# Bebra777228/PolGen-RVC

Hardware: AMD Instinct MI355X
Metric: real-time-factor (audio-sec/wall-sec) per GPU, 30s@16kHz RMVPE->48kHz (higher is better)
Workload: dtype f32 (conv products as 3 fp16 MFMAs of a hi/lo split, fp32 accumulate; fp32 elsewhere)

## Files before the change

polgen-rvc_amd/csrc/api_ops.hip:

```cpp
#include "api_internal.h"
#include "h3_device.h"

using namespace rvcx;
using namespace rvcx::api;

static void to_host(Ctx& c, float* h, const float* d, size_t n) {
  RVCX_HIP(hipMemcpyAsync(h, d, n * sizeof(float), hipMemcpyDeviceToHost, c.stream));
  RVCX_HIP(hipStreamSynchronize(c.stream));
}
#define TEMP_REGION(C) WeightRegion tmp_region_; RegionScope tmp_scope_(*(C), tmp_region_)

extern "C" {

int rvcx_op_conv1d(rvcx_ctx* ctx, const float* x, const float* w, const float* bias, const float* res,
                   float* y, int B, int Cin, int Tin, int Cout, int K, int stride, int dil,
                   int pad_left, int Tout, int groups, int pre_lrelu, float pre_slope, int act,
                   float act_slope, const int32_t* lens_in, const int32_t* lens_out) {
  API_BEGIN(ctx)
  TEMP_REGION(C);
  size_t nx = (size_t)B * Cin * Tin, ny = (size_t)B * Cout * Tout;
  C->arena.reserve((nx + 2 * ny) * 4 + (64 << 20));
  C->arena.reset();
  ConvW L = make_conv(*C, w, bias, Cout, Cin / groups, K, groups, true);
  float* dx = to_dev(*C, x, nx);
// ... 409 lines not shown
  for (size_t r = 0; r < (size_t)B * Cout * 2 * H; ++r)
    if (yp[r * Wpo] != 0.f || yp[r * Wpo + Wpo - 1] != 0.f) fail("convT2d: pad column not zero");
  unpad_rows(yp, y, (size_t)B * Cout, 2 * H, 2 * W);
  C->arena.reset();
  API_END
}

int rvcx_op_attention(rvcx_ctx* ctx, const float* q, const float* k, const float* v, float* out, int B, int H,
                      int D, int T, float scale, const float* emb_rel_k, const float* emb_rel_v, int window,
                      const int32_t* lens) {
  API_BEGIN(ctx)
  const size_t n = (size_t)B * H * D * T;
  C->arena.reserve(n * 16 + (attention_scratch_floats(B, H, T, window) + attention_split_floats(B, H, T)) * 4 + (64 << 20));
  C->arena.reset();
  float *dq = to_dev(*C, q, n), *dk = to_dev(*C, k, n), *dv = to_dev(*C, v, n);
  float* dout = C->arena.alloc<float>(n);
  float *ek = nullptr, *ev = nullptr, *scratch = nullptr;
  if (emb_rel_k) {
    ek = to_dev(*C, emb_rel_k, (size_t)(2 * window + 1) * D);
    ev = to_dev(*C, emb_rel_v, (size_t)(2 * window + 1) * D);
    scratch = C->arena.alloc<float>(attention_scratch_floats(B, H, T, window));
  }
  launch_attention(dq, dk, dv, dout, B, H, D, T, T, (long)H * D * T, (long)H * D * T, scale, ek, ev, window,
                   (lens ? to_dev(*C, lens, B) : nullptr), scratch, C->arena.alloc<float>(attention_split_floats(B, H, T)), C->stream);
  to_host(*C, out, dout, n);
  C->arena.reset();
  API_END
}

static void decode_xs(const std::vector<uint16_t>& raw, long rows, int Cc, float* out) {
  for (long r = 0; r < rows; ++r)
    for (int c = 0; c < Cc; ++c) {
      const size_t e = ((size_t)r * Cc * 2) + (size_t)(c >> 4) * 32 + ((c >> 3) & 1) * 8 + (c & 7);
      out[(size_t)r * Cc + c] = half_to_float(raw[e]) + half_to_float(raw[e + 16]) / 256.f;
    }
}

static void decode_split_cf(const std::vector<uint16_t>& raw, int B, int Cc, int T, float* out) {
  for (int b = 0; b < B; ++b)
    for (int c = 0; c < Cc; ++c)
      for (int t = 0; t < T; ++t) {
        const size_t item = (size_t)b * Cc * T * 2;
        const size_t hi = item + ((size_t)(((c >> 4) * 2 + 0) * 2 + ((c >> 3) & 1)) * T + t) * 8 + (c & 7);
        const size_t lo = item + ((size_t)(((c >> 4) * 2 + 1) * 2 + ((c >> 3) & 1)) * T + t) * 8 + (c & 7);
        out[((size_t)b * Cc + c) * T + t] = half_to_float(raw[hi]) + half_to_float(raw[lo]) / kH3Scale;
      }
}
// ... 445 lines not shown
```

polgen-rvc_amd/csrc/attention.hip:

```cpp
#include <cstdlib>

#include "conv.h"
#include "conv_device.h"
#include "ops.h"

namespace rvcx {

constexpr int KT = 32;
constexpr int VROW = 33;

template <int DT>
__global__ __launch_bounds__(256) void attn_kernel(const float* __restrict__ q, const float* __restrict__ k,
                                                   const float* __restrict__ v, float* __restrict__ out,
                                                   float* __restrict__ m_out, float* __restrict__ l_out,
                                                   const float* __restrict__ relq, int H, int D, int T,
                                                   int ld, long in_bs, long out_bs, float scale, int window,
                                                   const int* lens, int nsplit, float* opart) {
  __shared__ float Ks[32 * DT * KT];
  __shared__ float Vs[32 * DT * VROW];
  const int tid = threadIdx.x, lane = tid & 63, wave = tid >> 6;
  const int i = lane & 31, h = lane >> 5;
  const int b = blockIdx.z, hd = blockIdx.y;
  const int qblk = blockIdx.x / nsplit, split = blockIdx.x - qblk * nsplit;
  const int q0 = qblk * 128 + wave * 32;
  const int len = lens ? lens[b] : T;
  const long base = (long)b * in_bs + (long)hd * D * ld;
  const long obase = (long)b * out_bs + (long)hd * D * ld;
  const float* qb = q + base;
  const float* kb = k + base;
  const float* vb = v + base;
  const int nsteps = D / 2;

  float qreg[16 * DT];
  const int qi = q0 + i;
#pragma unroll
  for (int s = 0; s < 16 * DT; ++s) {
    float val = 0.f;
    if (s < nsteps && qi < T) val = qb[(long)(2 * s + h) * ld + qi] * scale;
    qreg[s] = val;
  }

  f32x16 acc_o[DT];
#pragma unroll
  for (int dt = 0; dt < DT; ++dt)
#pragma unroll
    for (int r = 0; r < 16; ++r) acc_o[dt][r] = 0.f;
  float m_run = -INFINITY, l_run = 0.f;
  const int nrel = 2 * window + 1;
  const float* relrow = relq ? relq + (((long)b * H + hd) * T + min(qi, T - 1)) * nrel : nullptr;

  const int tiles = (len + KT - 1) / KT;
  const int klo = (int)((long)tiles * split / nsplit) * KT;
  const int khi = min(len, (int)((long)tiles * (split + 1) / nsplit) * KT);
  for (int k0 = klo; k0 < khi; k0 += KT) {
    __syncthreads();
    for (int idx = tid; idx < 32 * DT * KT; idx += 256) {
      const int d = idx / KT, kk = idx % KT;
      const int key = k0 + kk;
      float kv = 0.f, vv = 0.f;
      if (d < D && key < len) {
        kv = kb[(long)d * ld + key];
        vv = vb[(long)d * ld + key];
      }
      Ks[d * KT + kk] = kv;
      Vs[d * VROW + kk] = vv;
    }
    __syncthreads();
    f32x16 sacc;
#pragma unroll
    for (int r = 0; r < 16; ++r) sacc[r] = 0.f;
#pragma unroll
    for (int s = 0; s < 16 * DT; ++s) {
      if (s < nsteps) {
        const float a = Ks[(2 * s + h) * KT + i];
        sacc = __builtin_amdgcn_mfma_f32_32x32x2f32(a, qreg[s], sacc, 0, 0, 0);
      }
    }
    const bool band = relq && (k0 <= q0 + 31 + window) && (k0 + KT - 1 >= q0 - window);
    float mloc = -INFINITY;
#pragma unroll
    for (int r = 0; r < 16; ++r) {
      const int key = k0 + (r & 3) + 8 * (r >> 2) + 4 * h;
      float sv = sacc[r];
      if (band) {
        const int rel = key - qi + window;
        if (rel >= 0 && rel < nrel && qi < T) sv += relrow[rel];
      }
      if (key >= len) sv = -INFINITY;
      sacc[r] = sv;
      mloc = fmaxf(mloc, sv);
    }
    const float mtile = fmaxf(mloc, __shfl_xor(mloc, 32));
    const float m_new = fmaxf(m_run, mtile);
    const float alpha = (m_run == -INFINITY) ? 0.f : expf(m_run - m_new);
    float lloc = 0.f;
#pragma unroll
    for (int r = 0; r < 16; ++r) {
      const float p = (sacc[r] == -INFINITY) ? 0.f : expf(sacc[r] - m_new);
      sacc[r] = p;
      lloc += p;
    }
    l_run = l_run * alpha + lloc + __shfl_xor(lloc, 32);
    m_run = m_new;
#pragma unroll
    for (int dt = 0; dt < DT; ++dt)
#pragma unroll
      for (int r = 0; r < 16; ++r) acc_o[dt][r] *= alpha;
#pragma unroll
    for (int s = 0; s < 16; ++s) {
      const int kidx = (s & 3) + 8 * (s >> 2) + 4 * h;
#pragma unroll
      for (int dt = 0; dt < DT; ++dt) {
        const float a = Vs[(dt * 32 + i) * VROW + kidx];
        acc_o[dt] = __builtin_amdgcn_mfma_f32_32x32x2f32(a, sacc[s], acc_o[dt], 0, 0, 0);
      }
    }
  }
  if (nsplit > 1) {
    if (qi < T) {
      const int DP = 32 * DT;
      float* pb = opart + (((long)b * H + hd) * nsplit + split) * (DP + 2) * T;
#pragma unroll
      for (int dt = 0; dt < DT; ++dt)
#pragma unroll
        for (int r = 0; r < 16; ++r) {
          const int d = dt * 32 + (r & 3) + 8 * (r >> 2) + 4 * h;
          pb[(long)d * T + qi] = acc_o[dt][r];
        }
      if (h == 0) {
        pb[(long)DP * T + qi] = m_run;
        pb[(long)(DP + 1) * T + qi] = l_run;
      }
    }
    return;
  }
  if (qi < T) {
    const float inv = 1.f / l_run;
    float* ob = out + obase;
#pragma unroll
    for (int dt = 0; dt < DT; ++dt)
#pragma unroll
      for (int r = 0; r < 16; ++r) {
        const int d = dt * 32 + (r & 3) + 8 * (r >> 2) + 4 * h;
        if (d < D) ob[(long)d * ld + qi] = (qi < len) ? acc_o[dt][r] * inv : 0.f;
      }
    if (m_out && h == 0) {
      m_out[((long)b * H + hd) * T + qi] = m_run;
      l_out[((long)b * H + hd) * T + qi] = l_run;
    }
  }
}

typedef _Float16 ahalf8 __attribute__((ext_vector_type(8)));
constexpr float kAttS = 256.f;
#ifndef RVCX_ATT_ABL
#define RVCX_ATT_ABL 0
#endif
constexpr int kAttAbl = RVCX_ATT_ABL;
__device__ __forceinline__ f32x16 att_mfma(ahalf8 a, ahalf8 b, f32x16 c) {
#if defined(__HIP_DEVICE_COMPILE__)
  return __builtin_amdgcn_mfma_f32_32x32x16_f16(a, b, c, 0, 0, 0);
#else
  return c;
#endif
}

struct AttRsrc {
#if defined(__HIP_DEVICE_COMPILE__)
  __amdgpu_buffer_rsrc_t r;
#endif
};
__device__ __forceinline__ AttRsrc att_rsrc(const float* base, int bytes) {
  AttRsrc b;
#if defined(__HIP_DEVICE_COMPILE__)
  b.r = __builtin_amdgcn_make_buffer_rsrc(const_cast<float*>(base), 0, bytes, 0x00020000);
#endif
  return b;
}
__device__ __forceinline__ float att_load(const AttRsrc& b, int off) {
#if defined(__HIP_DEVICE_COMPILE__)
  return __builtin_bit_cast(float, __builtin_amdgcn_raw_buffer_load_b32(b.r, off, 0, 0));
// ... 35 lines not shown
    ko[((s * 2 + 1) * 2 + hh) * 32 + key] = __builtin_bit_cast(uint4, a2);
  }
  for (int e0 = tid; e0 < V_ELEMS; e0 += 256) {
    const int dd = e0 & 31, hh = (e0 >> 5) & 1, s2 = (e0 >> 6) & 1, dt = e0 >> 7;
    const int d = dt * 32 + dd;
    ahalf8 a0, a2;
#pragma unroll
    for (int e = 0; e < 8; ++e) {
      const int r = 8 * s2 + e;
      const int key = k0 + (r & 3) + 8 * (r >> 2) + 4 * hh;
      const float val = (d < D && key < len) ? vb[(long)d * ld + key] : 0.f;
      ovf |= !(fabsf(val) < kH3ActLimit / kAttS);
      const _Float16 vh = (_Float16)val;
      a0[e] = (_Float16)((float)vh * kAttS);
      a2[e] = (_Float16)((val - (float)vh) * kAttS);
    }
    vo[(((dt * 2 + s2) * 2 + 0) * 2 + hh) * 32 + dd] = __builtin_bit_cast(uint4, a0);
    vo[(((dt * 2 + s2) * 2 + 1) * 2 + hh) * 32 + dd] = __builtin_bit_cast(uint4, a2);
  }
  if (ovf) report_h3_overflow(ovf_word, ovf_layer, seq);
}

typedef unsigned att_u32x4 __attribute__((ext_vector_type(4)));
template <int NKE, int NVE>
__device__ __forceinline__ void att_fetch(att_u32x4 (&rk)[NKE], att_u32x4 (&rv)[NVE], const uint4* __restrict__ kp,
                                          const uint4* __restrict__ vp, int tid) {
#pragma unroll
  for (int j = 0; j < NKE; ++j) rk[j] = *reinterpret_cast<const att_u32x4*>(kp + tid + 256 * j);
#pragma unroll
  for (int j = 0; j < NVE; ++j) rv[j] = *reinterpret_cast<const att_u32x4*>(vp + tid + 256 * j);
}
template <int NKE, int NVE>
__device__ __forceinline__ void att_commit(const att_u32x4 (&rk)[NKE], const att_u32x4 (&rv)[NVE], uint4* Ks, uint4* Vs,
                                           int tid) {
#pragma unroll
  for (int j = 0; j < NKE; ++j) *reinterpret_cast<att_u32x4*>(Ks + tid + 256 * j) = rk[j];
#pragma unroll
  for (int j = 0; j < NVE; ++j) *reinterpret_cast<att_u32x4*>(Vs + tid + 256 * j) = rv[j];
}

template <int DT>
__global__ __launch_bounds__(256, 2) void attn_h3_kernel(const float* __restrict__ q, const uint4* __restrict__ kimg,
                                                      const uint4* __restrict__ vimg, float* __restrict__ out,
                                                      float* __restrict__ m_out, float* __restrict__ l_out,
                                                      const float* __restrict__ relq, int H, int D, int T,
                                                      int ld, long in_bs, long out_bs, float scale, int window,
                                                      const int* lens, int nsplit, float* opart, int* ovf_word,
                                                      int* ovf_layer, int seq) {
  constexpr int NS = 2 * DT;
  __shared__ uint4 Ks[NS * 2 * 2 * 32];
  __shared__ uint4 Vs[DT * 2 * 2 * 2 * 32];
  const int tid = threadIdx.x, lane = tid & 63, wave = tid >> 6;
  const int i = lane & 31, h = lane >> 5;
  const int b = blockIdx.z, hd = blockIdx.y;
  const int qblk = blockIdx.x / nsplit, split = blockIdx.x - qblk * nsplit;
  const int q0 = qblk * 128 + wave * 32;
  const int len = lens ? lens[b] : T;
  const long base = (long)b * in_bs + (long)hd * D * ld;
  const long obase = (long)b * out_bs + (long)hd * D * ld;
  const float* qb = q + base;

  bool ovf = false;
  ahalf8 qh[NS], ql[NS];
  const int qi = q0 + i;
#pragma unroll
  for (int s = 0; s < NS; ++s)
#pragma unroll
    for (int e = 0; e < 8; ++e) {
      const int d = 16 * s + 8 * h + e;
      const float val = (d < D && qi < T) ? qb[(long)d * ld + qi] * scale : 0.f;
      ovf |= !(fabsf(val) < kH3ActLimit);
      const _Float16 vh = (_Float16)val;
      qh[s][e] = vh;
      ql[s][e] = (_Float16)((val - (float)vh) * kAttS);
    }

  f32x16 acc_o[DT];
#pragma unroll
  for (int dt = 0; dt < DT; ++dt)
#pragma unroll
    for (int r = 0; r < 16; ++r) acc_o[dt][r] = 0.f;
  float m_run = -INFINITY, l_run = 0.f;
  const int nrel = 2 * window + 1;
  const float* relrow = relq ? relq + (((long)b * H + hd) * T + min(qi, T - 1)) * nrel : nullptr;

  constexpr float invS = 1.f / kAttS;
  constexpr int KSZ = NS * 2 * 2 * 32, VSZ = DT * 2 * 2 * 2 * 32;
  constexpr int NKE = KSZ / 256, NVE = VSZ / 256;
  static_assert(KSZ % 256 == 0 && VSZ % 256 == 0, "image sizes are multiples of the workgroup");
  const int ntile = (T + 31) / 32;
  const uint4* kt_base = kimg + ((long)b * H + hd) * ntile * KSZ;
  const uint4* vt_base = vimg + ((long)b * H + hd) * ntile * VSZ;
  att_u32x4 rk[NKE], rv[NVE];
  auto fetch = [&](int k0) {
    att_fetch<NKE, NVE>(rk, rv, kt_base + (long)(k0 >> 5) * KSZ, vt_base + (long)(k0 >> 5) * VSZ, tid);
  };
  auto commit = [&]() { att_commit<NKE, NVE>(rk, rv, Ks, Vs, tid); };

  const int tiles = (len + 31) / 32;
  const int klo = (int)((long)tiles * split / nsplit) * 32;
  const int khi = min(len, (int)((long)tiles * (split + 1) / nsplit) * 32);
  if (klo < khi) fetch(klo);
  for (int k0 = klo; k0 < khi; k0 += 32) {
    if (!(kAttAbl & 16)) __syncthreads();
    if (!(kAttAbl & 4) || k0 == klo) commit();
    __syncthreads();
    if (k0 + 32 < khi && !(kAttAbl & 2)) fetch(k0 + 32);
    f32x16 sacc;
#pragma unroll
    for (int r = 0; r < 16; ++r) sacc[r] = 0.f;
#pragma unroll
    for (int s = 0; s < NS; ++s) {
      if (16 * s < D) {
        const ahalf8 a0 = __builtin_bit_cast(ahalf8, Ks[((s * 2 + 0) * 2 + h) * 32 + i]);
        const ahalf8 a2 = __builtin_bit_cast(ahalf8, Ks[((s * 2 + 1) * 2 + h) * 32 + i]);
        const ahalf8 a1 = a0 * (_Float16)invS;
        if (kAttAbl & 1) {
          sacc[s] += (float)a0[0] + (float)a2[1] + (float)a1[2];
          continue;
        }
        sacc = att_mfma(a0, qh[s], sacc);
        sacc = att_mfma(a1, ql[s], sacc);
        sacc = att_mfma(a2, qh[s], sacc);
      }
    }
    const bool band = relq && (k0 <= q0 + 31 + window) && (k0 + 31 >= q0 - window);
    const bool edge = band || k0 + 32 > len;
    float mloc = -INFINITY;
    if (edge) {
#pragma unroll
      for (int r = 0; r < 16; ++r) {
        const int key = k0 + (r & 3) + 8 * (r >> 2) + 4 * h;
        float sv = sacc[r] * invS;
        if (band) {
          const int rel = key - qi + window;
          if (rel >= 0 && rel < nrel && qi < T) sv += relrow[rel];
        }
        if (key >= len) sv = -INFINITY;
        sacc[r] = sv;
        mloc = fmaxf(mloc, sv);
      }
    } else {
#pragma unroll
      for (int r = 0; r < 16; ++r) {
        sacc[r] *= invS;
        mloc = fmaxf(mloc, sacc[r]);
      }
    }
    const float mtile = fmaxf(mloc, __shfl_xor(mloc, 32));
    const float m_new = fmaxf(m_run, mtile);
    const float alpha = (m_run == -INFINITY) ? 0.f : __expf(m_run - m_new);
    float lloc = 0.f;
    ahalf8 ph[2], pl[2];
#pragma unroll
    for (int r = 0; r < 16; ++r) {
      float p = (kAttAbl & 8) ? sacc[r] - m_new : __expf(sacc[r] - m_new);
      if (edge) p = (sacc[r] == -INFINITY) ? 0.f : p;
      lloc += p;
      const _Float16 vh = (_Float16)p;
      ph[r >> 3][r & 7] = vh;
      pl[r >> 3][r & 7] = (_Float16)((p - (float)vh) * kAttS);
    }
    l_run = l_run * alpha + lloc + __shfl_xor(lloc, 32);
    m_run = m_new;
#pragma unroll
    for (int dt = 0; dt < DT; ++dt)
#pragma unroll
      for (int r = 0; r < 16; ++r) acc_o[dt][r] *= alpha;
#pragma unroll
    for (int dt = 0; dt < DT; ++dt)
#pragma unroll
      for (int s2 = 0; s2 < 2; ++s2) {
        const ahalf8 a0 = __builtin_bit_cast(ahalf8, Vs[(((dt * 2 + s2) * 2 + 0) * 2 + h) * 32 + i]);
        const ahalf8 a2 = __builtin_bit_cast(ahalf8, Vs[(((dt * 2 + s2) * 2 + 1) * 2 + h) * 32 + i]);
        const ahalf8 a1 = a0 * (_Float16)invS;
        if (kAttAbl & 1) {
          acc_o[dt][s2] += (float)a0[0] + (float)a2[1] + (float)a1[2] + (float)ph[s2][0] + (float)pl[s2][1];
          continue;
        }
        acc_o[dt] = att_mfma(a0, ph[s2], acc_o[dt]);
        acc_o[dt] = att_mfma(a1, pl[s2], acc_o[dt]);
        acc_o[dt] = att_mfma(a2, ph[s2], acc_o[dt]);
      }
  }
  if (ovf) report_h3_overflow(ovf_word, ovf_layer, seq);
#pragma unroll
  for (int dt = 0; dt < DT; ++dt)
#pragma unroll
    for (int r = 0; r < 16; ++r) acc_o[dt][r] *= invS;
  if (nsplit > 1) {
    if (qi < T) {
      const int DP = 32 * DT;
      float* pb = opart + (((long)b * H + hd) * nsplit + split) * (DP + 2) * T;
#pragma unroll
      for (int dt = 0; dt < DT; ++dt)
#pragma unroll
        for (int r = 0; r < 16; ++r) {
          const int d = dt * 32 + (r & 3) + 8 * (r >> 2) + 4 * h;
          pb[(long)d * T + qi] = acc_o[dt][r];
        }
      if (h == 0) {
        pb[(long)DP * T + qi] = m_run;
        pb[(long)(DP + 1) * T + qi] = l_run;
      }
    }
    return;
  }
  if (qi < T) {
    const float inv = 1.f / l_run;
    float* ob = out + obase;
#pragma unroll
    for (int dt = 0; dt < DT; ++dt)
#pragma unroll
      for (int r = 0; r < 16; ++r) {
        const int d = dt * 32 + (r & 3) + 8 * (r >> 2) + 4 * h;
        if (d < D) ob[(long)d * ld + qi] = (qi < len) ? acc_o[dt][r] * inv : 0.f;
      }
    if (m_out && h == 0) {
      m_out[((long)b * H + hd) * T + qi] = m_run;
      l_out[((long)b * H + hd) * T + qi] = l_run;
    }
  }
}


__global__ __launch_bounds__(256) void attn_merge_kernel(const float* __restrict__ opart, float* __restrict__ out,
                                                         float* m_out, float* l_out, int H, int D, int DP, int T, int ld,
                                                         long out_bs, int nsplit, const int* lens) {
  const int t = blockIdx.x * 64 + (threadIdx.x & 63), part = threadIdx.x >> 6;
  const int hd = blockIdx.y >> 2, dq = blockIdx.y & 3, b = blockIdx.z;
  if (t >= T) return;
  const float* pb = opart + (((long)b * H + hd) * nsplit) * (DP + 2) * T;
  const long ss = (long)(DP + 2) * T;
  float ms[8], w[8];
  float m = -INFINITY, l = 0.f;
#pragma unroll
  for (int s = 0; s < 8; ++s) {
    ms[s] = s < nsplit ? pb[s * ss + (long)DP * T + t] : -INFINITY;
    m = fmaxf(m, ms[s]);
  }
#pragma unroll
  for (int s = 0; s < 8; ++s) {
    w[s] = (ms[s] == -INFINITY) ? 0.f : expf(ms[s] - m);
    if (s < nsplit) l += w[s] * pb[s * ss + (long)(DP + 1) * T + t];
  }
  const int len = lens ? lens[b] : T;
  const float inv = 1.f / l;
  float* ob = out + (long)b * out_bs + (long)hd * D * ld;
  const int dper = (D + 3) / 4, d0 = dq * dper, d1 = min(D, d0 + dper);
  for (int d = d0 + part; d < d1; d += 4) {
    float acc = 0.f;
#pragma unroll
    for (int s = 0; s < 8; ++s)
      if (s < nsplit) acc += w[s] * pb[s * ss + (long)d * T + t];
    ob[(long)d * ld + t] = t < len ? acc * inv : 0.f;
  }
  if (m_out && part == 0 && dq == 0) {
    m_out[((long)b * H + hd) * T + t] = m;
    l_out[((long)b * H + hd) * T + t] = l;
  }
}

__global__ __launch_bounds__(256) void rel_logits_kernel(const float* __restrict__ q, const float* __restrict__ ek,
                                                         float* __restrict__ relq, int H, int D, int T, int ld,
                                                         long in_bs, float scale, int nrel) {
  extern __shared__ float eks[];
  for (int idx = threadIdx.x; idx < nrel * D; idx += 256) eks[idx] = ek[idx];
  __syncthreads();
  const int tq = threadIdx.x & 63, part = __builtin_amdgcn_readfirstlane(threadIdx.x >> 6);
  const int nmine = part < nrel ? (nrel - part + 3) / 4 : 0;
  const int t = blockIdx.x * 64 + tq;
  const int hd = blockIdx.y, b = blockIdx.z;
  if (t >= T) return;
  const float* qb = q + (long)b * in_bs + (long)hd * D * ld;
  float acc[8];
#pragma unroll
  for (int i = 0; i < 8; ++i) acc[i] = 0.f;
  int d = 0;
  for (; d + 8 <= D; d += 8) {
    float qv[8];
#pragma unroll
    for (int u = 0; u < 8; ++u) qv[u] = qb[(long)(d + u) * ld + t] * scale;
#pragma unroll
    for (int i = 0; i < 8; ++i)
      if (i < nmine) {
        const float* e = eks + (part + 4 * i) * D + d;
        if ((D & 3) == 0) {
          const float4 e0 = *reinterpret_cast<const float4*>(e), e1 = *reinterpret_cast<const float4*>(e + 4);
          acc[i] = fmaf(qv[0], e0.x, acc[i]);
          acc[i] = fmaf(qv[1], e0.y, acc[i]);
          acc[i] = fmaf(qv[2], e0.z, acc[i]);
          acc[i] = fmaf(qv[3], e0.w, acc[i]);
          acc[i] = fmaf(qv[4], e1.x, acc[i]);
          acc[i] = fmaf(qv[5], e1.y, acc[i]);
          acc[i] = fmaf(qv[6], e1.z, acc[i]);
          acc[i] = fmaf(qv[7], e1.w, acc[i]);
        } else {
#pragma unroll
          for (int u = 0; u < 8; ++u) acc[i] = fmaf(qv[u], e[u], acc[i]);
        }
      }
  }
  for (; d < D; ++d) {
    const float qv = qb[(long)d * ld + t] * scale;
#pragma unroll
    for (int i = 0; i < 8; ++i)
      if (i < nmine) acc[i] = fmaf(qv, eks[(part + 4 * i) * D + d], acc[i]);
  }
  float* o = relq + (((long)b * H + hd) * T + t) * nrel;
#pragma unroll
  for (int i = 0; i < 8; ++i) {
    const int r = part + 4 * i;
    if (r < nrel) o[r] = acc[i];
  }
}

__global__ __launch_bounds__(256) void rel_values_kernel(const float* __restrict__ q, const float* __restrict__ k,
                                                         const float* __restrict__ relq,
                                                         const float* __restrict__ m_in,
                                                         const float* __restrict__ l_in,
                                                         const float* __restrict__ ev, float* __restrict__ out,
                                                         int H, int D, int T, int ld, long in_bs, long out_bs, float scale,
                                                         int window, const int* lens) {
  extern __shared__ float sm[];
  const int nrel = 2 * window + 1;
  const int KW = 32 + 2 * window;
  float* evs = sm;
  float* ps = evs + nrel * D;
  float* qs = ps + 32 * (nrel + 1);
  float* ks = qs + D * 32;
  const int tq = threadIdx.x & 31, part = threadIdx.x >> 5;
  const int hd = blockIdx.y, b = blockIdx.z;
  const int tb = blockIdx.x * 32;
  const int t = tb + tq;
  const int len = lens ? lens[b] : T;
  const long base = (long)b * in_bs + (long)hd * D * ld;
  const long obase = (long)b * out_bs + (long)hd * D * ld;
  for (int idx = threadIdx.x; idx < nrel * D; idx += 256) evs[idx] = ev[idx];
  for (int idx = threadIdx.x; idx < D * 32; idx += 256) {
    const int d = idx >> 5, j = idx & 31;
    qs[idx] = tb + j < T ? q[base + (long)d * ld + tb + j] * scale : 0.f;
  }
  for (int idx = threadIdx.x; idx < D * KW; idx += 256) {
    const int d = idx / KW, j = idx - d * KW;
    const int key = tb - window + j;
    ks[idx] = (key >= 0 && key < T) ? k[base + (long)d * ld + key] : 0.f;
  }
  __syncthreads();
  if (t < T) {
    const float m = m_in[((long)b * H + hd) * T + t], l = l_in[((long)b * H + hd) * T + t];
    for (int r = part; r < nrel; r += 8) {
      const int key = t + r - window;
      float p = 0.f;
      if (key >= 0 && key < len) {
        float s = 0.f;
        for (int d = 0; d < D; ++d) s = fmaf(qs[d * 32 + tq], ks[d * KW + tq + r], s);
        s += relq[(((long)b * H + hd) * T + t) * nrel + r];
        p = expf(s - m) / l;
      }
      ps[tq * (nrel + 1) + r] = p;
    }
  }
  __syncthreads();
  if (t < T && t < len) {
    for (int d = part; d < D; d += 8) {
      float acc = 0.f;
      for (int r = 0; r < nrel; ++r) acc = fmaf(ps[tq * (nrel + 1) + r], evs[r * D + d], acc);
      out[obase + (long)d * ld + t] += acc;
    }
  }
}

void launch_attention(const float* q, const float* k, const float* v, float* out, int B, int H, int D, int T,
                      int ld, long in_bs, long out_bs, float scale, const float* emb_rel_k, const float* emb_rel_v, int window,
                      const int* lens, float* scratch, float* split_scratch, hipStream_t stream, int* ovf, int* ovf_layer,
                      int seq, bool allow_h3) {
  RVCX_CHECK(D % 2 == 0 && D <= 96, "attention: head dim must be even and <= 96");
  const int nrel = 2 * window + 1;
  float *relq = nullptr, *mb = nullptr, *lb = nullptr;
  if (emb_rel_k) {
    RVCX_CHECK(nrel <= 32 && scratch != nullptr, "attention: window too large / no scratch");
    relq = scratch;
    mb = relq + (size_t)B * H * T * nrel;
    lb = mb + (size_t)B * H * T;
    hipLaunchKernelGGL(rel_logits_kernel, dim3(cdiv(T, 64), H, B), dim3(256), nrel * D * sizeof(float), stream,
                       q, emb_rel_k, relq, H, D, T, ld, in_bs, scale, nrel);
  }
  const int DT = cdiv(D, 32);
  const long blocks = (long)cdiv(T, 128) * H;
  (void)B;
  int nsplit = 1;
  static const int max_split = std::min(8, getenv("RVCX_ATT_MAXSPLIT") ? atoi(getenv("RVCX_ATT_MAXSPLIT")) : 8);
  static const int want_blocks = getenv("RVCX_ATT_BLOCKS") ? atoi(getenv("RVCX_ATT_BLOCKS")) : 200;
  static const int min_keys = getenv("RVCX_ATT_MINKEYS") ? atoi(getenv("RVCX_ATT_MINKEYS")) : 256;
  while (nsplit < max_split && blocks * nsplit < want_blocks && T / (nsplit * 2) >= min_keys) nsplit *= 2;
  float* opart = nullptr;
  if (nsplit > 1) {
    if (split_scratch) opart = split_scratch;
    else nsplit = 1;
  }
  float* mo = nsplit > 1 ? nullptr : mb;
  float* lo = nsplit > 1 ? nullptr : lb;
  dim3 grid(cdiv(T, 128) * nsplit, H, B);
  static const int h3_env = getenv("RVCX_ATT_H3") ? atoi(getenv("RVCX_ATT_H3")) : 1;
  const int h3 = h3_env && !g_force_fp32 && allow_h3;
  if (h3) {
    RVCX_CHECK(split_scratch != nullptr, "attention: the split-fp16 kernel needs its scratch");
    const int ntile = cdiv(T, 32);
    uint4* kimg = reinterpret_cast<uint4*>(split_scratch + (size_t)B * H * 8 * 98 * T);
    uint4* vimg = kimg + (size_t)B * H * ntile * (DT * 256);
    const dim3 pg(ntile, H, B);
    if (DT == 1) {
      hipLaunchKernelGGL(att_presplit_kernel<1>, pg, dim3(256), 0, stream, k, v, kimg, vimg, H, D, T, ld, in_bs, lens, ovf, ovf_layer, seq);
      hipLaunchKernelGGL(attn_h3_kernel<1>, grid, dim3(256), 0, stream, q, kimg, vimg, out, mo, lo, relq, H, D, T, ld, in_bs,
                         out_bs, scale, window, lens, nsplit, opart, ovf, ovf_layer, seq);
    } else if (DT == 2) {
      hipLaunchKernelGGL(att_presplit_kernel<2>, pg, dim3(256), 0, stream, k, v, kimg, vimg, H, D, T, ld, in_bs, lens, ovf, ovf_layer, seq);
      hipLaunchKernelGGL(attn_h3_kernel<2>, grid, dim3(256), 0, stream, q, kimg, vimg, out, mo, lo, relq, H, D, T, ld, in_bs,
                         out_bs, scale, window, lens, nsplit, opart, ovf, ovf_layer, seq);
    } else {
      hipLaunchKernelGGL(att_presplit_kernel<3>, pg, dim3(256), 0, stream, k, v, kimg, vimg, H, D, T, ld, in_bs, lens, ovf, ovf_layer, seq);
      hipLaunchKernelGGL(attn_h3_kernel<3>, grid, dim3(256), 0, stream, q, kimg, vimg, out, mo, lo, relq, H, D, T, ld, in_bs,
                         out_bs, scale, window, lens, nsplit, opart, ovf, ovf_layer, seq);
    }
  }
  else if (DT == 1)
    hipLaunchKernelGGL(attn_kernel<1>, grid, dim3(256), 0, stream, q, k, v, out, mo, lo, relq, H, D, T, ld, in_bs,
                       out_bs, scale, window, lens, nsplit, opart);
  else if (DT == 2)
    hipLaunchKernelGGL(attn_kernel<2>, grid, dim3(256), 0, stream, q, k, v, out, mo, lo, relq, H, D, T, ld, in_bs,
                       out_bs, scale, window, lens, nsplit, opart);
  else
    hipLaunchKernelGGL(attn_kernel<3>, grid, dim3(256), 0, stream, q, k, v, out, mo, lo, relq, H, D, T, ld, in_bs,
                       out_bs, scale, window, lens, nsplit, opart);
  if (nsplit > 1)
    hipLaunchKernelGGL(attn_merge_kernel, dim3(cdiv(T, 64), H * 4, B), dim3(256), 0, stream, opart, out, mb, lb, H, D,
                       32 * DT, T, ld, out_bs, nsplit, lens);
  if (emb_rel_v) {
    size_t lds = ((size_t)nrel * D + 32 * (nrel + 1) + (size_t)D * 32 + (size_t)D * (32 + 2 * window)) * sizeof(float);
    hipLaunchKernelGGL(rel_values_kernel, dim3(cdiv(T, 32), H, B), dim3(256), lds, stream, q, k, relq, mb, lb,
                       emb_rel_v, out, H, D, T, ld, in_bs, out_bs, scale, window, lens);
  }
  RVCX_HIP(hipGetLastError());
}

size_t attention_scratch_floats(int B, int H, int T, int window) {
  return (size_t)B * H * T * (2 * window + 1) + 2 * (size_t)B * H * T;
}

size_t attention_split_floats(int B, int H, int T) { return (size_t)B * H * (8 * 98 * (size_t)T + 2 * 96 * ((size_t)T + 32)); }

double attention_flops(int B, int H, int D, int T) { return 4.0 * B * H * (double)T * T * D; }

}
```

Baseline: 1262.

## Fuse relative-value attention into merge and split key tiles across wave groups

The attention kernels now write the banded relative-position logits to scratch, and the split-merge kernel applies the relative-value term from them. This replaces the separate rel_values_kernel, which recomputed the q·k band and needed the m/l outputs. For DT==3 with few blocks, an extra wave group processes alternate key tiles and merges its softmax state through LDS, giving more waves per block without more splits. Debug ablation switches are removed, and the merge kernel now always runs when relative values are present.

```diff
diff --git a/polgen-rvc_amd/csrc/api_ops.hip b/polgen-rvc_amd/csrc/api_ops.hip
--- a/polgen-rvc_amd/csrc/api_ops.hip
+++ b/polgen-rvc_amd/csrc/api_ops.hip
@@ -455,7 +455,8 @@
     scratch = C->arena.alloc<float>(attention_scratch_floats(B, H, T, window));
   }
   launch_attention(dq, dk, dv, dout, B, H, D, T, T, (long)H * D * T, (long)H * D * T, scale, ek, ev, window,
-                   (lens ? to_dev(*C, lens, B) : nullptr), scratch, C->arena.alloc<float>(attention_split_floats(B, H, T)), C->stream);
+                   (lens ? to_dev(*C, lens, B) : nullptr), scratch, C->arena.alloc<float>(attention_split_floats(B, H, T)), C->stream,
+                   C->dev_err);
   to_host(*C, out, dout, n);
   C->arena.reset();
   API_END
diff --git a/polgen-rvc_amd/csrc/attention.hip b/polgen-rvc_amd/csrc/attention.hip
--- a/polgen-rvc_amd/csrc/attention.hip
+++ b/polgen-rvc_amd/csrc/attention.hip
@@ -12,10 +12,9 @@
 template <int DT>
 __global__ __launch_bounds__(256) void attn_kernel(const float* __restrict__ q, const float* __restrict__ k,
                                                    const float* __restrict__ v, float* __restrict__ out,
-                                                   float* __restrict__ m_out, float* __restrict__ l_out,
-                                                   const float* __restrict__ relq, int H, int D, int T,
-                                                   int ld, long in_bs, long out_bs, float scale, int window,
-                                                   const int* lens, int nsplit, float* opart) {
+                                                   const float* __restrict__ relq, float* __restrict__ band_out,
+                                                   int H, int D, int T, int ld, long in_bs, long out_bs, float scale,
+                                                   int window, const int* lens, int nsplit, float* opart) {
   __shared__ float Ks[32 * DT * KT];
   __shared__ float Vs[32 * DT * VROW];
   const int tid = threadIdx.x, lane = tid & 63, wave = tid >> 6;
@@ -48,6 +47,7 @@
   float m_run = -INFINITY, l_run = 0.f;
   const int nrel = 2 * window + 1;
   const float* relrow = relq ? relq + (((long)b * H + hd) * T + min(qi, T - 1)) * nrel : nullptr;
+  float* bandrow = band_out ? band_out + (((long)b * H + hd) * T + min(qi, T - 1)) * nrel : nullptr;
 
   const int tiles = (len + KT - 1) / KT;
   const int klo = (int)((long)tiles * split / nsplit) * KT;
@@ -82,11 +82,11 @@
     for (int r = 0; r < 16; ++r) {
       const int key = k0 + (r & 3) + 8 * (r >> 2) + 4 * h;
       float sv = sacc[r];
-      if (band) {
-        const int rel = key - qi + window;
-        if (rel >= 0 && rel < nrel && qi < T) sv += relrow[rel];
-      }
+      const int rel = key - qi + window;
+      const bool inband = band && rel >= 0 && rel < nrel && qi < T;
+      if (inband) sv += relrow[rel];
       if (key >= len) sv = -INFINITY;
+      if (inband && bandrow) bandrow[rel] = sv;
       sacc[r] = sv;
       mloc = fmaxf(mloc, sv);
     }
@@ -116,7 +116,7 @@
       }
     }
   }
-  if (nsplit > 1) {
+  if (opart) {
     if (qi < T) {
       const int DP = 32 * DT;
       float* pb = opart + (((long)b * H + hd) * nsplit + split) * (DP + 2) * T;
@@ -144,19 +144,11 @@
         const int d = dt * 32 + (r & 3) + 8 * (r >> 2) + 4 * h;
         if (d < D) ob[(long)d * ld + qi] = (qi < len) ? acc_o[dt][r] * inv : 0.f;
       }
-    if (m_out && h == 0) {
-      m_out[((long)b * H + hd) * T + qi] = m_run;
-      l_out[((long)b * H + hd) * T + qi] = l_run;
-    }
   }
 }
 
 typedef _Float16 ahalf8 __attribute__((ext_vector_type(8)));
 constexpr float kAttS = 256.f;
-#ifndef RVCX_ATT_ABL
-#define RVCX_ATT_ABL 0
-#endif
-constexpr int kAttAbl = RVCX_ATT_ABL;
 __device__ __forceinline__ f32x16 att_mfma(ahalf8 a, ahalf8 b, f32x16 c) {
 #if defined(__HIP_DEVICE_COMPILE__)
   return __builtin_amdgcn_mfma_f32_32x32x16_f16(a, b, c, 0, 0, 0);
@@ -238,39 +230,45 @@
 }
 
 typedef unsigned att_u32x4 __attribute__((ext_vector_type(4)));
-template <int NKE, int NVE>
+template <int NKE, int NVE, int NT>
 __device__ __forceinline__ void att_fetch(att_u32x4 (&rk)[NKE], att_u32x4 (&rv)[NVE], const uint4* __restrict__ kp,
-                                          const uint4* __restrict__ vp, int tid) {
-#pragma unroll
-  for (int j = 0; j < NKE; ++j) rk[j] = *reinterpret_cast<const att_u32x4*>(kp + tid + 256 * j);
-#pragma unroll
-  for (int j = 0; j < NVE; ++j) rv[j] = *reinterpret_cast<const att_u32x4*>(vp + tid + 256 * j);
-}
-template <int NKE, int NVE>
+                                          const uint4* __restrict__ vp, int tid, int klast, int vlast) {
+#pragma unroll
+  for (int j = 0; j < NKE; ++j) rk[j] = *reinterpret_cast<const att_u32x4*>(kp + min(tid + NT * j, klast));
+#pragma unroll
+  for (int j = 0; j < NVE; ++j) rv[j] = *reinterpret_cast<const att_u32x4*>(vp + min(tid + NT * j, vlast));
+}
+template <int NKE, int NVE, int NT>
 __device__ __forceinline__ void att_commit(const att_u32x4 (&rk)[NKE], const att_u32x4 (&rv)[NVE], uint4* Ks, uint4* Vs,
                                            int tid) {
 #pragma unroll
-  for (int j = 0; j < NKE; ++j) *reinterpret_cast<att_u32x4*>(Ks + tid + 256 * j) = rk[j];
-#pragma unroll
-  for (int j = 0; j < NVE; ++j) *reinterpret_cast<att_u32x4*>(Vs + tid + 256 * j) = rv[j];
-}
-
-template <int DT>
-__global__ __launch_bounds__(256, 2) void attn_h3_kernel(const float* __restrict__ q, const uint4* __restrict__ kimg,
+  for (int j = 0; j < NKE; ++j) *reinterpret_cast<att_u32x4*>(Ks + tid + NT * j) = rk[j];
+#pragma unroll
+  for (int j = 0; j < NVE; ++j) *reinterpret_cast<att_u32x4*>(Vs + tid + NT * j) = rv[j];
+}
+
+template <int DT, int NQW, int NG>
+__global__ __launch_bounds__(NQW * NG * 64, 2) void attn_h3_kernel(const float* __restrict__ q, const uint4* __restrict__ kimg,
                                                       const uint4* __restrict__ vimg, float* __restrict__ out,
-                                                      float* __restrict__ m_out, float* __restrict__ l_out,
-                                                      const float* __restrict__ relq, int H, int D, int T,
-                                                      int ld, long in_bs, long out_bs, float scale, int window,
-                                                      const int* lens, int nsplit, float* opart, int* ovf_word,
+                                                      const float* __restrict__ relq, float* __restrict__ band_out,
+                                                      int H, int D, int T, int ld, long in_bs, long out_bs, float scale,
+                                                      int window, const int* lens, int nsplit, float* opart, int* ovf_word,
                                                       int* ovf_layer, int seq) {
   constexpr int NS = 2 * DT;
-  __shared__ uint4 Ks[NS * 2 * 2 * 32];
-  __shared__ uint4 Vs[DT * 2 * 2 * 2 * 32];
-  const int tid = threadIdx.x, lane = tid & 63, wave = tid >> 6;
+  constexpr int NT = NQW * NG * 64;
+  constexpr int KSZ = NS * 2 * 2 * 32;
+  constexpr int VSZ = DT * 2 * 2 * 2 * 32;
+  __shared__ uint4 stage[NG * (KSZ + VSZ)];
+  __shared__ float xml[NG == 2 ? NQW * 2 * 64 : 1];
+  static_assert(NG == 1 || (NG == 2 && NQW * DT * 256 <= NG * (KSZ + VSZ)), "group 1's accumulators fit the staging area");
+  uint4* const Ks = stage;
+  uint4* const Vs = stage + NG * KSZ;
+  const int tid = threadIdx.x, lane = tid & 63, wave = __builtin_amdgcn_readfirstlane(tid >> 6);
+  const int grp = (NG == 2 && wave >= NQW) ? 1 : 0, qw = wave - grp * NQW;
   const int i = lane & 31, h = lane >> 5;
   const int b = blockIdx.z, hd = blockIdx.y;
   const int qblk = blockIdx.x / nsplit, split = blockIdx.x - qblk * nsplit;
-  const int q0 = qblk * 128 + wave * 32;
+  const int q0 = qblk * (32 * NQW) + qw * 32;
   const int len = lens ? lens[b] : T;
   const long base = (long)b * in_bs + (long)hd * D * ld;
   const long obase = (long)b * out_bs + (long)hd * D * ld;
@@ -299,42 +297,44 @@
   float m_run = -INFINITY, l_run = 0.f;
   const int nrel = 2 * window + 1;
   const float* relrow = relq ? relq + (((long)b * H + hd) * T + min(qi, T - 1)) * nrel : nullptr;
+  float* bandrow = band_out ? band_out + (((long)b * H + hd) * T + min(qi, T - 1)) * nrel : nullptr;
 
   constexpr float invS = 1.f / kAttS;
-  constexpr int KSZ = NS * 2 * 2 * 32, VSZ = DT * 2 * 2 * 2 * 32;
-  constexpr int NKE = KSZ / 256, NVE = VSZ / 256;
-  static_assert(KSZ % 256 == 0 && VSZ % 256 == 0, "image sizes are multiples of the workgroup");
+  constexpr int NKE = NG * KSZ / NT, NVE = NG * VSZ / NT;
+  static_assert((NG * KSZ) % NT == 0 && (NG * VSZ) % NT == 0, "a stage's images are multiples of the workgroup");
   const int ntile = (T + 31) / 32;
   const uint4* kt_base = kimg + ((long)b * H + hd) * ntile * KSZ;
   const uint4* vt_base = vimg + ((long)b * H + hd) * ntile * VSZ;
+  const int tiles = (len + 31) / 32;
+  const int tlo = (int)((long)tiles * split / nsplit);
+  const int thi = (int)((long)tiles * (split + 1) / nsplit);
   att_u32x4 rk[NKE], rv[NVE];
-  auto fetch = [&](int k0) {
-    att_fetch<NKE, NVE>(rk, rv, kt_base + (long)(k0 >> 5) * KSZ, vt_base + (long)(k0 >> 5) * VSZ, tid);
-  };
-  auto commit = [&]() { att_commit<NKE, NVE>(rk, rv, Ks, Vs, tid); };
-
-  const int tiles = (len + 31) / 32;
-  const int klo = (int)((long)tiles * split / nsplit) * 32;
-  const int khi = min(len, (int)((long)tiles * (split + 1) / nsplit) * 32);
-  if (klo < khi) fetch(klo);
-  for (int k0 = klo; k0 < khi; k0 += 32) {
-    if (!(kAttAbl & 16)) __syncthreads();
-    if (!(kAttAbl & 4) || k0 == klo) commit();
+  if (tlo < thi) {
+    const int nv = min(NG, thi - tlo);
+    att_fetch<NKE, NVE, NT>(rk, rv, kt_base + (long)tlo * KSZ, vt_base + (long)tlo * VSZ, tid, nv * KSZ - 1, nv * VSZ - 1);
+  }
+  const uint4* const Kt = Ks + grp * KSZ;
+  const uint4* const Vt = Vs + grp * VSZ;
+  for (int t0 = tlo; t0 < thi; t0 += NG) {
     __syncthreads();
-    if (k0 + 32 < khi && !(kAttAbl & 2)) fetch(k0 + 32);
+    att_commit<NKE, NVE, NT>(rk, rv, Ks, Vs, tid);
+    __syncthreads();
+    if (t0 + NG < thi) {
+      const int nv = min(NG, thi - t0 - NG);
+      att_fetch<NKE, NVE, NT>(rk, rv, kt_base + (long)(t0 + NG) * KSZ, vt_base + (long)(t0 + NG) * VSZ, tid, nv * KSZ - 1,
+                              nv * VSZ - 1);
+    }
+    if (NG == 2 && t0 + grp >= thi) continue;
+    const int k0 = (t0 + grp) * 32;
     f32x16 sacc;
 #pragma unroll
     for (int r = 0; r < 16; ++r) sacc[r] = 0.f;
 #pragma unroll
     for (int s = 0; s < NS; ++s) {
       if (16 * s < D) {
-        const ahalf8 a0 = __builtin_bit_cast(ahalf8, Ks[((s * 2 + 0) * 2 + h) * 32 + i]);
-        const ahalf8 a2 = __builtin_bit_cast(ahalf8, Ks[((s * 2 + 1) * 2 + h) * 32 + i]);
+        const ahalf8 a0 = __builtin_bit_cast(ahalf8, Kt[((s * 2 + 0) * 2 + h) * 32 + i]);
+        const ahalf8 a2 = __builtin_bit_cast(ahalf8, Kt[((s * 2 + 1) * 2 + h) * 32 + i]);
         const ahalf8 a1 = a0 * (_Float16)invS;
-        if (kAttAbl & 1) {
-          sacc[s] += (float)a0[0] + (float)a2[1] + (float)a1[2];
-          continue;
-        }
         sacc = att_mfma(a0, qh[s], sacc);
         sacc = att_mfma(a1, ql[s], sacc);
         sacc = att_mfma(a2, qh[s], sacc);
@@ -348,11 +348,11 @@
       for (int r = 0; r < 16; ++r) {
         const int key = k0 + (r & 3) + 8 * (r >> 2) + 4 * h;
         float sv = sacc[r] * invS;
-        if (band) {
-          const int rel = key - qi + window;
-          if (rel >= 0 && rel < nrel && qi < T) sv += relrow[rel];
-        }
+        const int rel = key - qi + window;
+        const bool inband = band && rel >= 0 && rel < nrel && qi < T;
+        if (inband) sv += relrow[rel];
         if (key >= len) sv = -INFINITY;
+        if (inband && bandrow) bandrow[rel] = sv;
         sacc[r] = sv;
         mloc = fmaxf(mloc, sv);
       }
@@ -370,7 +370,7 @@
     ahalf8 ph[2], pl[2];
 #pragma unroll
     for (int r = 0; r < 16; ++r) {
-      float p = (kAttAbl & 8) ? sacc[r] - m_new : __expf(sacc[r] - m_new);
+      float p = __expf(sacc[r] - m_new);
       if (edge) p = (sacc[r] == -INFINITY) ? 0.f : p;
       lloc += p;
       const _Float16 vh = (_Float16)p;
@@ -387,13 +387,9 @@
     for (int dt = 0; dt < DT; ++dt)
 #pragma unroll
       for (int s2 = 0; s2 < 2; ++s2) {
-        const ahalf8 a0 = __builtin_bit_cast(ahalf8, Vs[(((dt * 2 + s2) * 2 + 0) * 2 + h) * 32 + i]);
-        const ahalf8 a2 = __builtin_bit_cast(ahalf8, Vs[(((dt * 2 + s2) * 2 + 1) * 2 + h) * 32 + i]);
+        const ahalf8 a0 = __builtin_bit_cast(ahalf8, Vt[(((dt * 2 + s2) * 2 + 0) * 2 + h) * 32 + i]);
+        const ahalf8 a2 = __builtin_bit_cast(ahalf8, Vt[(((dt * 2 + s2) * 2 + 1) * 2 + h) * 32 + i]);
         const ahalf8 a1 = a0 * (_Float16)invS;
-        if (kAttAbl & 1) {
-          acc_o[dt][s2] += (float)a0[0] + (float)a2[1] + (float)a1[2] + (float)ph[s2][0] + (float)pl[s2][1];
-          continue;
-        }
         acc_o[dt] = att_mfma(a0, ph[s2], acc_o[dt]);
         acc_o[dt] = att_mfma(a1, pl[s2], acc_o[dt]);
         acc_o[dt] = att_mfma(a2, ph[s2], acc_o[dt]);
@@ -404,7 +400,51 @@
   for (int dt = 0; dt < DT; ++dt)
 #pragma unroll
     for (int r = 0; r < 16; ++r) acc_o[dt][r] *= invS;
-  if (nsplit > 1) {
+  if constexpr (NG == 2) {
+  typedef float att_f32x4 __attribute__((ext_vector_type(4)));
+  att_f32x4* const xo = reinterpret_cast<att_f32x4*>(stage) + (long)qw * DT * 4 * 64 + lane;
+  __syncthreads();
+  if (grp == 1) {
+#pragma unroll
+    for (int dt = 0; dt < DT; ++dt)
+#pragma unroll
+      for (int c = 0; c < 4; ++c) {
+        att_f32x4 o;
+#pragma unroll
+        for (int e = 0; e < 4; ++e) o[e] = acc_o[dt][4 * c + e];
+        xo[(dt * 4 + c) * 64] = o;
+      }
+    xml[(qw * 2 + 0) * 64 + lane] = m_run;
+    xml[(qw * 2 + 1) * 64 + lane] = l_run;
+  }
+  __syncthreads();
+  if (grp == 1) return;
+  {
+    const float m1 = xml[(qw * 2 + 0) * 64 + lane], l1 = xml[(qw * 2 + 1) * 64 + lane];
+    const float m = fmaxf(m_run, m1);
+    const float w0 = (m_run == -INFINITY) ? 0.f : expf(m_run - m);
+    const float w1 = (m1 == -INFINITY) ? 0.f : expf(m1 - m);
+    float l = 0.f;
+    l += w0 * l_run;
+    l += w1 * l1;
+#pragma unroll
+    for (int dt = 0; dt < DT; ++dt)
+#pragma unroll
+      for (int c = 0; c < 4; ++c) {
+        const att_f32x4 o = xo[(dt * 4 + c) * 64];
+#pragma unroll
+        for (int e = 0; e < 4; ++e) {
+          float acc = 0.f;
+          acc += w0 * acc_o[dt][4 * c + e];
+          acc += w1 * o[e];
+          acc_o[dt][4 * c + e] = acc;
+        }
+      }
+    m_run = m;
+    l_run = l;
+  }
+  }
+  if (opart) {
     if (qi < T) {
       const int DP = 32 * DT;
       float* pb = opart + (((long)b * H + hd) * nsplit + split) * (DP + 2) * T;
@@ -432,19 +472,31 @@
         const int d = dt * 32 + (r & 3) + 8 * (r >> 2) + 4 * h;
         if (d < D) ob[(long)d * ld + qi] = (qi < len) ? acc_o[dt][r] * inv : 0.f;
       }
-    if (m_out && h == 0) {
-      m_out[((long)b * H + hd) * T + qi] = m_run;
-      l_out[((long)b * H + hd) * T + qi] = l_run;
-    }
-  }
-}
-
-
-__global__ __launch_bounds__(256) void attn_merge_kernel(const float* __restrict__ opart, float* __restrict__ out,
-                                                         float* m_out, float* l_out, int H, int D, int DP, int T, int ld,
-                                                         long out_bs, int nsplit, const int* lens) {
-  const int t = blockIdx.x * 64 + (threadIdx.x & 63), part = threadIdx.x >> 6;
+  }
+}
+
+
+__global__ __launch_bounds__(256) void attn_merge_kernel(const float* __restrict__ opart, float* __restrict__ out, int H,
+                                                         int D, int DP, int T, int ld, long out_bs, int nsplit,
+                                                         const int* lens, const float* __restrict__ band,
+                                                         const float* __restrict__ ev, int nrel) {
+  extern __shared__ float msm[];
+  const int tq = threadIdx.x & 63, part = threadIdx.x >> 6;
+  const int t = blockIdx.x * 64 + tq;
   const int hd = blockIdx.y >> 2, dq = blockIdx.y & 3, b = blockIdx.z;
+  const int dper = (D + 3) / 4, d0 = dq * dper, d1 = min(D, d0 + dper);
+  float* evs = msm;
+  float* bs = msm + nrel * dper;
+  if (band) {
+    for (int idx = threadIdx.x; idx < nrel * dper; idx += 256) {
+      const int r = idx / dper, d = d0 + idx - r * dper;
+      evs[idx] = d < d1 ? ev[r * D + d] : 0.f;
+    }
+    const float* bb = band + (((long)b * H + hd) * T + (long)blockIdx.x * 64) * nrel;
+    const int nb = min(64, T - blockIdx.x * 64) * nrel;
+    for (int idx = threadIdx.x; idx < nb; idx += 256) bs[idx] = bb[idx];
+    __syncthreads();
+  }
   if (t >= T) return;
   const float* pb = opart + (((long)b * H + hd) * nsplit) * (DP + 2) * T;
   const long ss = (long)(DP + 2) * T;
@@ -462,24 +514,31 @@
   }
   const int len = lens ? lens[b] : T;
   const float inv = 1.f / l;
+  float p[32];
+#pragma unroll
+  for (int r = 0; r < 32; ++r) p[r] = (band && r < nrel) ? expf(bs[tq * nrel + r] - m) / l : 0.f;
   float* ob = out + (long)b * out_bs + (long)hd * D * ld;
-  const int dper = (D + 3) / 4, d0 = dq * dper, d1 = min(D, d0 + dper);
   for (int d = d0 + part; d < d1; d += 4) {
     float acc = 0.f;
 #pragma unroll
     for (int s = 0; s < 8; ++s)
       if (s < nsplit) acc += w[s] * pb[s * ss + (long)d * T + t];
-    ob[(long)d * ld + t] = t < len ? acc * inv : 0.f;
-  }
-  if (m_out && part == 0 && dq == 0) {
-    m_out[((long)b * H + hd) * T + t] = m;
-    l_out[((long)b * H + hd) * T + t] = l;
+    float o = acc * inv;
+    if (band) {
+      float ra = 0.f;
+#pragma unroll
+      for (int r = 0; r < 32; ++r)
+        if (r < nrel) ra = fmaf(p[r], evs[r * dper + d - d0], ra);
+      o += ra;
+    }
+    ob[(long)d * ld + t] = t < len ? o : 0.f;
   }
 }
 
 __global__ __launch_bounds__(256) void rel_logits_kernel(const float* __restrict__ q, const float* __restrict__ ek,
-                                                         float* __restrict__ relq, int H, int D, int T, int ld,
-                                                         long in_bs, float scale, int nrel) {
+                                                         float* __restrict__ relq, float* __restrict__ band, int H,
+                                                         int D, int T, int ld, long in_bs, float scale, int nrel,
+                                                         int window, const int* lens) {
   extern __shared__ float eks[];
   for (int idx = threadIdx.x; idx < nrel * D; idx += 256) eks[idx] = ek[idx];
   __syncthreads();
@@ -524,65 +583,15 @@
       if (i < nmine) acc[i] = fmaf(qv, eks[(part + 4 * i) * D + d], acc[i]);
   }
   float* o = relq + (((long)b * H + hd) * T + t) * nrel;
+  float* bo = band ? band + (((long)b * H + hd) * T + t) * nrel : nullptr;
+  const int len = lens ? lens[b] : T;
 #pragma unroll
   for (int i = 0; i < 8; ++i) {
     const int r = part + 4 * i;
-    if (r < nrel) o[r] = acc[i];
-  }
-}
-
-__global__ __launch_bounds__(256) void rel_values_kernel(const float* __restrict__ q, const float* __restrict__ k,
-                                                         const float* __restrict__ relq,
-                                                         const float* __restrict__ m_in,
-                                                         const float* __restrict__ l_in,
-                                                         const float* __restrict__ ev, float* __restrict__ out,
-                                                         int H, int D, int T, int ld, long in_bs, long out_bs, float scale,
-                                                         int window, const int* lens) {
-  extern __shared__ float sm[];
-  const int nrel = 2 * window + 1;
-  const int KW = 32 + 2 * window;
-  float* evs = sm;
-  float* ps = evs + nrel * D;
-  float* qs = ps + 32 * (nrel + 1);
-  float* ks = qs + D * 32;
-  const int tq = threadIdx.x & 31, part = threadIdx.x >> 5;
-  const int hd = blockIdx.y, b = blockIdx.z;
-  const int tb = blockIdx.x * 32;
-  const int t = tb + tq;
-  const int len = lens ? lens[b] : T;
-  const long base = (long)b * in_bs + (long)hd * D * ld;
-  const long obase = (long)b * out_bs + (long)hd * D * ld;
-  for (int idx = threadIdx.x; idx < nrel * D; idx += 256) evs[idx] = ev[idx];
-  for (int idx = threadIdx.x; idx < D * 32; idx += 256) {
-    const int d = idx >> 5, j = idx & 31;
-    qs[idx] = tb + j < T ? q[base + (long)d * ld + tb + j] * scale : 0.f;
-  }
-  for (int idx = threadIdx.x; idx < D * KW; idx += 256) {
-    const int d = idx / KW, j = idx - d * KW;
-    const int key = tb - window + j;
-    ks[idx] = (key >= 0 && key < T) ? k[base + (long)d * ld + key] : 0.f;
-  }
-  __syncthreads();
-  if (t < T) {
-    const float m = m_in[((long)b * H + hd) * T + t], l = l_in[((long)b * H + hd) * T + t];
-    for (int r = part; r < nrel; r += 8) {
+    if (r < nrel) {
+      o[r] = acc[i];
       const int key = t + r - window;
-      float p = 0.f;
-      if (key >= 0 && key < len) {
-        float s = 0.f;
-        for (int d = 0; d < D; ++d) s = fmaf(qs[d * 32 + tq], ks[d * KW + tq + r], s);
-        s += relq[(((long)b * H + hd) * T + t) * nrel + r];
-        p = expf(s - m) / l;
-      }
-      ps[tq * (nrel + 1) + r] = p;
-    }
-  }
-  __syncthreads();
-  if (t < T && t < len) {
-    for (int d = part; d < D; d += 8) {
-      float acc = 0.f;
-      for (int r = 0; r < nrel; ++r) acc = fmaf(ps[tq * (nrel + 1) + r], evs[r * D + d], acc);
-      out[obase + (long)d * ld + t] += acc;
+      if (bo && (key < 0 || key >= len)) bo[r] = -INFINITY;
     }
   }
 }
@@ -593,76 +602,76 @@
                       int seq, bool allow_h3) {
   RVCX_CHECK(D % 2 == 0 && D <= 96, "attention: head dim must be even and <= 96");
   const int nrel = 2 * window + 1;
-  float *relq = nullptr, *mb = nullptr, *lb = nullptr;
+  float *relq = nullptr, *band = nullptr;
   if (emb_rel_k) {
     RVCX_CHECK(nrel <= 32 && scratch != nullptr, "attention: window too large / no scratch");
     relq = scratch;
-    mb = relq + (size_t)B * H * T * nrel;
-    lb = mb + (size_t)B * H * T;
+    if (emb_rel_v) band = relq + (size_t)B * H * T * nrel;
     hipLaunchKernelGGL(rel_logits_kernel, dim3(cdiv(T, 64), H, B), dim3(256), nrel * D * sizeof(float), stream,
-                       q, emb_rel_k, relq, H, D, T, ld, in_bs, scale, nrel);
+                       q, emb_rel_k, relq, band, H, D, T, ld, in_bs, scale, nrel, window, lens);
+  } else {
+    RVCX_CHECK(!emb_rel_v, "attention: relative-position values without the keys' embedding");
   }
   const int DT = cdiv(D, 32);
-  const long blocks = (long)cdiv(T, 128) * H;
+  static const int h3_env = getenv("RVCX_ATT_H3") ? atoi(getenv("RVCX_ATT_H3")) : 1;
+  const int h3 = h3_env && !g_force_fp32 && allow_h3;
+  constexpr int nqw = 4;
+  const long blocks = (long)cdiv(T, 32 * nqw) * H;
   (void)B;
   int nsplit = 1;
+  const bool two_groups = h3 && DT == 3 && blocks < 128;
   static const int max_split = std::min(8, getenv("RVCX_ATT_MAXSPLIT") ? atoi(getenv("RVCX_ATT_MAXSPLIT")) : 8);
-  static const int want_blocks = getenv("RVCX_ATT_BLOCKS") ? atoi(getenv("RVCX_ATT_BLOCKS")) : 200;
+  static const int want_env = getenv("RVCX_ATT_BLOCKS") ? atoi(getenv("RVCX_ATT_BLOCKS")) : 0;
+  const int want_blocks = want_env ? want_env : (two_groups ? 128 : 200);
   static const int min_keys = getenv("RVCX_ATT_MINKEYS") ? atoi(getenv("RVCX_ATT_MINKEYS")) : 256;
   while (nsplit < max_split && blocks * nsplit < want_blocks && T / (nsplit * 2) >= min_keys) nsplit *= 2;
-  float* opart = nullptr;
-  if (nsplit > 1) {
-    if (split_scratch) opart = split_scratch;
-    else nsplit = 1;
-  }
-  float* mo = nsplit > 1 ? nullptr : mb;
-  float* lo = nsplit > 1 ? nullptr : lb;
-  dim3 grid(cdiv(T, 128) * nsplit, H, B);
-  static const int h3_env = getenv("RVCX_ATT_H3") ? atoi(getenv("RVCX_ATT_H3")) : 1;
-  const int h3 = h3_env && !g_force_fp32 && allow_h3;
+  if (!split_scratch) nsplit = 1;
+  const bool merge = nsplit > 1 || band != nullptr;
+  RVCX_CHECK(!merge || split_scratch != nullptr, "attention: the merge needs the split scratch");
+  float* opart = merge ? split_scratch : nullptr;
   if (h3) {
     RVCX_CHECK(split_scratch != nullptr, "attention: the split-fp16 kernel needs its scratch");
     const int ntile = cdiv(T, 32);
     uint4* kimg = reinterpret_cast<uint4*>(split_scratch + (size_t)B * H * 8 * 98 * T);
     uint4* vimg = kimg + (size_t)B * H * ntile * (DT * 256);
     const dim3 pg(ntile, H, B);
-    if (DT == 1) {
-      hipLaunchKernelGGL(att_presplit_kernel<1>, pg, dim3(256), 0, stream, k, v, kimg, vimg, H, D, T, ld, in_bs, lens, ovf, ovf_layer, seq);
-      hipLaunchKernelGGL(attn_h3_kernel<1>, grid, dim3(256), 0, stream, q, kimg, vimg, out, mo, lo, relq, H, D, T, ld, in_bs,
-                         out_bs, scale, window, lens, nsplit, opart, ovf, ovf_layer, seq);
-    } else if (DT == 2) {
-      hipLaunchKernelGGL(att_presplit_kernel<2>, pg, dim3(256), 0, stream, k, v, kimg, vimg, H, D, T, ld, in_bs, lens, ovf, ovf_layer, seq);
-      hipLaunchKernelGGL(attn_h3_kernel<2>, grid, dim3(256), 0, stream, q, kimg, vimg, out, mo, lo, relq, H, D, T, ld, in_bs,
-                         out_bs, scale, window, lens, nsplit, opart, ovf, ovf_layer, seq);
-    } else {
-      hipLaunchKernelGGL(att_presplit_kernel<3>, pg, dim3(256), 0, stream, k, v, kimg, vimg, H, D, T, ld, in_bs, lens, ovf, ovf_layer, seq);
-      hipLaunchKernelGGL(attn_h3_kernel<3>, grid, dim3(256), 0, stream, q, kimg, vimg, out, mo, lo, relq, H, D, T, ld, in_bs,
-                         out_bs, scale, window, lens, nsplit, opart, ovf, ovf_layer, seq);
-    }
-  }
-  else if (DT == 1)
-    hipLaunchKernelGGL(attn_kernel<1>, grid, dim3(256), 0, stream, q, k, v, out, mo, lo, relq, H, D, T, ld, in_bs,
-                       out_bs, scale, window, lens, nsplit, opart);
-  else if (DT == 2)
-    hipLaunchKernelGGL(attn_kernel<2>, grid, dim3(256), 0, stream, q, k, v, out, mo, lo, relq, H, D, T, ld, in_bs,
-                       out_bs, scale, window, lens, nsplit, opart);
-  else
-    hipLaunchKernelGGL(attn_kernel<3>, grid, dim3(256), 0, stream, q, k, v, out, mo, lo, relq, H, D, T, ld, in_bs,
-                       out_bs, scale, window, lens, nsplit, opart);
-  if (nsplit > 1)
-    hipLaunchKernelGGL(attn_merge_kernel, dim3(cdiv(T, 64), H * 4, B), dim3(256), 0, stream, opart, out, mb, lb, H, D,
-                       32 * DT, T, ld, out_bs, nsplit, lens);
-  if (emb_rel_v) {
-    size_t lds = ((size_t)nrel * D + 32 * (nrel + 1) + (size_t)D * 32 + (size_t)D * (32 + 2 * window)) * sizeof(float);
-    hipLaunchKernelGGL(rel_values_kernel, dim3(cdiv(T, 32), H, B), dim3(256), lds, stream, q, k, relq, mb, lb,
-                       emb_rel_v, out, H, D, T, ld, in_bs, out_bs, scale, window, lens);
+    const dim3 grid(cdiv(T, 32 * nqw) * nsplit, H, B);
+#define RVCX_ATT_H3(DT_, NG_)                                                                                               \
+  hipLaunchKernelGGL((attn_h3_kernel<DT_, nqw, NG_>), grid, dim3(nqw * NG_ * 64), 0, stream, q, kimg, vimg, out, relq, band, \
+                     H, D, T, ld, in_bs, out_bs, scale, window, lens, nsplit, opart, ovf, ovf_layer, seq)
+#define RVCX_ATT_LAUNCH(DT_, NG_)                                                                                           \
+  do {                                                                                                                      \
+    hipLaunchKernelGGL(att_presplit_kernel<DT_>, pg, dim3(256), 0, stream, k, v, kimg, vimg, H, D, T, ld, in_bs, lens, ovf,  \
+                       ovf_layer, seq);                                                                                     \
+    RVCX_ATT_H3(DT_, NG_);                                                                                                  \
+  } while (0)
+    if (DT == 1) RVCX_ATT_LAUNCH(1, 1);
+    else if (DT == 2) RVCX_ATT_LAUNCH(2, 1);
+    else if (two_groups) RVCX_ATT_LAUNCH(3, 2);
+    else RVCX_ATT_LAUNCH(3, 1);
+#undef RVCX_ATT_LAUNCH
+#undef RVCX_ATT_H3
+  } else {
+    const dim3 grid(cdiv(T, 128) * nsplit, H, B);
+    if (DT == 1)
+      hipLaunchKernelGGL(attn_kernel<1>, grid, dim3(256), 0, stream, q, k, v, out, relq, band, H, D, T, ld, in_bs, out_bs,
+                         scale, window, lens, nsplit, opart);
+    else if (DT == 2)
+      hipLaunchKernelGGL(attn_kernel<2>, grid, dim3(256), 0, stream, q, k, v, out, relq, band, H, D, T, ld, in_bs, out_bs,
+                         scale, window, lens, nsplit, opart);
+    else
+      hipLaunchKernelGGL(attn_kernel<3>, grid, dim3(256), 0, stream, q, k, v, out, relq, band, H, D, T, ld, in_bs, out_bs,
+                         scale, window, lens, nsplit, opart);
+  }
+  if (merge) {
+    const size_t lds = band ? ((size_t)nrel * cdiv(D, 4) + 64 * (size_t)nrel) * sizeof(float) : 0;
+    hipLaunchKernelGGL(attn_merge_kernel, dim3(cdiv(T, 64), H * 4, B), dim3(256), lds, stream, opart, out, H, D, 32 * DT, T,
+                       ld, out_bs, nsplit, lens, band, emb_rel_v, nrel);
   }
   RVCX_HIP(hipGetLastError());
 }
 
-size_t attention_scratch_floats(int B, int H, int T, int window) {
-  return (size_t)B * H * T * (2 * window + 1) + 2 * (size_t)B * H * T;
-}
+size_t attention_scratch_floats(int B, int H, int T, int window) { return 2 * (size_t)B * H * T * (2 * window + 1); }
 
 size_t attention_split_floats(int B, int H, int T) { return (size_t)B * H * (8 * 98 * (size_t)T + 2 * 96 * ((size_t)T + 32)); }
 
```

Result: no change. 1269 (median of 2 runs) (+0.5%).
